# zju3dv/pats

Measured on AMD Instinct MI355X. Metric: image-pairs/sec (coarse+fine OT) on 640x480 MegaDepth; OT iters/sec per pair, higher is better.
Workload: dtype f32 (contractions: fp32 operands split into fp16 hi + lo, three exact-product MFMA passes, fp32 accumulate)

## Files before the change

include/pats_amd.h:

```cpp
#ifndef PATS_AMD_H
#define PATS_AMD_H

#include <stddef.h>
#include <stdint.h>

#ifdef __cplusplus
extern "C" {
#endif

typedef void* pats_stream_t;

enum {
    PATS_OK = 0,
    PATS_ERR_INVALID = 1,
    PATS_ERR_UNSUPPORTED = 2,
    PATS_ERR_LAUNCH = 3,
    PATS_ERR_NO_DEVICE = 4
};

enum { PATS_SINKHORN_AUTO = 0, PATS_SINKHORN_LOG = 1, PATS_SINKHORN_KERNEL = 2 };

const char* pats_version(void);
#define PATS_ABI_VERSION 8
int pats_abi_version(void);
const char* pats_last_error(void);
int pats_device_count(void);
int pats_set_sinkhorn_mode(int mode);
int pats_set_fine_fused(int on);

int pats_set_third_gather(int mode);

int pats_sinkhorn_fallbacks(int64_t* count, int reset);

int pats_cost_f32(const float* d0, const float* d1, int64_t batch, int D, int n, int m, float* out,
                  pats_stream_t stream);

size_t pats_sinkhorn_workspace_bytes(int64_t batch, int M, int N);
int pats_sinkhorn_f32(const float* Z, int64_t batch, int M, int N, const float* log_mu,
                      const float* log_nu, int iters, float* out, void* workspace,
                      size_t workspace_bytes, pats_stream_t stream);

size_t pats_ot_workspace_bytes(int64_t batch, int M, int N);
int pats_log_optimal_transport_f32(const float* scores, int64_t batch, int m, int n,
                                   const float* alpha, const float* ns, int iters, float* Z,
                                   void* workspace, size_t workspace_bytes, pats_stream_t stream);

size_t pats_ot2_workspace_bytes(int64_t batch, int m, int n);
int pats_log_optimal_transport2_flags_f32(const float* scores, int64_t batch, int m, int n,
                                          const float* one, const float* ns, int iters, float bias_k,
                                          float* Z, uint8_t* col_nomatch, void* workspace,
                                          size_t workspace_bytes, pats_stream_t stream);
int pats_log_optimal_transport2_f32(const float* scores, int64_t batch, int m, int n,
                                    const float* one, const float* ns, int iters, float bias_k,
                                    float* Z, void* workspace, size_t workspace_bytes,
                                    pats_stream_t stream);

int pats_cost_ot_f32(const float* d0, const float* d1, int64_t batch, int D, int n, int m,
                     int variant, const float* scalar, const float* ns, int iters, float bias_k,
                     float* Z, void* workspace, size_t workspace_bytes, pats_stream_t stream);
size_t pats_cost_ot_workspace_bytes(int64_t batch, int D, int n, int m, int variant);
int pats_cost_ot_flags_f32(const float* d0, const float* d1, int64_t batch, int D, int n, int m,
                           int variant, const float* scalar, const float* ns, int iters, float bias_k,
                           float* Z, uint8_t* col_nomatch, void* workspace, size_t workspace_bytes,
                           pats_stream_t stream);

int pats_set_cost_ot_mid_event(void* event);

int pats_cost_ot_flags_counted_f32(const float* d0, const float* d1, int64_t batch_cap, const int64_t* batch_dev,
                                   int D, int n, int m, int variant, const float* scalar, const float* ns, int iters,
                                   float bias_k, float* Z, uint8_t* col_nomatch, void* workspace,
                                   size_t workspace_bytes, pats_stream_t stream);

int pats_colmass_sqrt_f32(const float* Z, int64_t batch, int M, int N, float* out,
                          pats_stream_t stream);
int pats_colmass_flags_f32(const float* Z, int64_t batch, int M, int N, float* out, uint8_t* col_nomatch,
                           pats_stream_t stream);
int pats_dustbin_bias_inplace_f32(float* Z, int64_t batch, int M, int N, float k,
                                  pats_stream_t stream);
int pats_exp_f32(const float* Z, int64_t count, float* out, pats_stream_t stream);

int pats_argmax_f32(const float* Z, int64_t batch, int M, int N, int64_t* row_arg,
                    int64_t* col_arg, pats_stream_t stream);

int pats_iterative_expand_f32(const float* P, int input_is_log, int64_t batch, int M, int N,
                              const float* scalex, const float* scaley, int lim3, int h, int w,
                              float lower_bound, int iter_num, float* whole_cost, float* core_cost,
                              float* average_point, float* x_scale, float* y_scale, int64_t* bound,
                              uint8_t* row_nomatch, pats_stream_t stream);

int pats_iterative_expand_counted_f32(const float* P, int input_is_log, int64_t batch_cap, const int64_t* batch_dev,
                                      int M, int N, const float* scalex, const float* scaley, int lim3, int h, int w,
                                      float lower_bound, int iter_num, float* whole_cost, float* core_cost,
                                      float* average_point, float* x_scale, float* y_scale, int64_t* bound,
                                      uint8_t* row_nomatch, pats_stream_t stream);

int pats_split_patches(const int32_t* sum_cycle_host, int height, int width, int max_once_used,
                       int64_t* second_layer_set, int64_t* third_layer_set);
int pats_split_patches_device(const int32_t* sum_cycle, int64_t pairs, int height, int width,
                              int max_once_used, int64_t* second_layer_set, int64_t* third_layer_set,
                              int32_t* cycle_num, pats_stream_t stream);

int pats_compute_imgs_bounds_f32(const float* x_scale, const float* y_scale,
                                 const float* average_point, const uint8_t* if_nomatching, int Np,
                                 int height, int width, int img, int64_t* bound5, int64_t* K_out,
                                 float* x_scale_new, float* y_scale_new, float* average_new,
                                 pats_stream_t stream);

int pats_left_crops_f32(const float* left, int n_img, int H, int W, const int64_t* bound5, int64_t K,
                        int height, int width, float* out, pats_stream_t stream);

int pats_compute_imgs_bounds_batch_f32(const float* x_scale, const float* y_scale, const float* average_point,
                                       const uint8_t* if_nomatching, int n_img, int Np, int height, int width,
                                       int64_t* bound5, int64_t* K_img, int64_t* K_total, float* x_scale_new,
// ... 372 lines not shown
```

pats_amd/_lib.py:

```python
import ctypes
import os

_HERE = os.path.dirname(os.path.abspath(__file__))
LIB_PATH = os.path.join(_HERE, "libpats_amd.so")
if os.environ.get("PATS_AMD_DIAG_LIB", "") not in ("", "0"):
    _sfx = os.environ["PATS_AMD_DIAG_LIB"]
    LIB_PATH = os.path.join(_HERE, "libpats_amd_diag%s.so" % ("" if _sfx == "1" else _sfx))

c_void_p, c_int, c_i64, c_f, c_size = (ctypes.c_void_p, ctypes.c_int, ctypes.c_int64, ctypes.c_float,
                                       ctypes.c_size_t)

ABI_VERSION = 8



class PairTable(ctypes.Structure):
    _fields_ = [("pairs", ctypes.c_int64), ("shape_host", c_void_p), ("cell_base_host", c_void_p), ("shape", c_void_p),
                ("cell_base", c_void_p), ("img_base", c_void_p)]


_TAB = ctypes.POINTER(PairTable)


class CropFormat(ctypes.Structure):
    _fields_ = [("dtype", ctypes.c_int32), ("layout", ctypes.c_int32), ("normalize", ctypes.c_int32),
                ("mean", ctypes.c_float * 3), ("std", ctypes.c_float * 3)]


_FMT = ctypes.POINTER(CropFormat)

SIGNATURES = {
    "pats_version": (ctypes.c_char_p, []),
    "pats_abi_version": (c_int, []),
    "pats_last_error": (ctypes.c_char_p, []),
    "pats_device_count": (c_int, []),
    "pats_set_sinkhorn_mode": (c_int, [c_int]),
    "pats_set_fine_fused": (c_int, [c_int]),
    "pats_set_third_gather": (c_int, [c_int]),
    "pats_sinkhorn_fallbacks": (c_int, [ctypes.POINTER(ctypes.c_int64), c_int]),
    "pats_set_gnn_redo_mode": (c_int, [c_int]),
    "pats_gnn_overflows": (c_int, [ctypes.POINTER(ctypes.c_int64), c_int]),
    "pats_cost_f32": (c_int, [c_void_p, c_void_p, c_i64, c_int, c_int, c_int, c_void_p, c_void_p]),
    "pats_sinkhorn_workspace_bytes": (c_size, [c_i64, c_int, c_int]),
    "pats_sinkhorn_f32": (c_int, [c_void_p, c_i64, c_int, c_int, c_void_p, c_void_p, c_int, c_void_p,
                                  c_void_p, c_size, c_void_p]),
    "pats_ot_workspace_bytes": (c_size, [c_i64, c_int, c_int]),
    "pats_log_optimal_transport_f32": (c_int, [c_void_p, c_i64, c_int, c_int, c_void_p, c_void_p, c_int,
                                               c_void_p, c_void_p, c_size, c_void_p]),
    "pats_ot2_workspace_bytes": (c_size, [c_i64, c_int, c_int]),
    "pats_log_optimal_transport2_f32": (c_int, [c_void_p, c_i64, c_int, c_int, c_void_p, c_void_p, c_int,
                                                c_f, c_void_p, c_void_p, c_size, c_void_p]),
    "pats_cost_ot_f32": (c_int, [c_void_p, c_void_p, c_i64, c_int, c_int, c_int, c_int, c_void_p,
                                 c_void_p, c_int, c_f, c_void_p, c_void_p, c_size, c_void_p]),
    "pats_cost_ot_flags_f32": (c_int, [c_void_p, c_void_p, c_i64, c_int, c_int, c_int, c_int, c_void_p,
                                       c_void_p, c_int, c_f, c_void_p, c_void_p, c_void_p, c_size, c_void_p]),
    "pats_set_cost_ot_mid_event": (c_int, [c_void_p]),
    "pats_cost_ot_flags_counted_f32": (c_int, [c_void_p, c_void_p, c_i64, c_void_p, c_int, c_int, c_int, c_int, c_void_p,
                                               c_void_p, c_int, c_f, c_void_p, c_void_p, c_void_p, c_size, c_void_p]),
    "pats_iterative_expand_counted_f32": (c_int, [c_void_p, c_int, c_i64, c_void_p, c_int, c_int, c_void_p, c_void_p, c_int,
                                                  c_int, c_int, c_f, c_int, c_void_p, c_void_p, c_void_p,
                                                  c_void_p, c_void_p, c_void_p, c_void_p, c_void_p]),
    "pats_fine_descriptors_counted_f32": (c_int, [c_void_p, c_void_p, c_void_p, c_void_p, c_void_p, c_i64, c_void_p, c_int,
                                                  c_void_p, c_void_p]),
    "pats_log_optimal_transport2_flags_f32": (c_int, [c_void_p, c_i64, c_int, c_int, c_void_p, c_void_p, c_int,
                                                      c_f, c_void_p, c_void_p, c_void_p, c_size, c_void_p]),
    "pats_colmass_flags_f32": (c_int, [c_void_p, c_i64, c_int, c_int, c_void_p, c_void_p, c_void_p]),
    "pats_cost_ot_workspace_bytes": (c_size, [c_i64, c_int, c_int, c_int, c_int]),
    "pats_colmass_sqrt_f32": (c_int, [c_void_p, c_i64, c_int, c_int, c_void_p, c_void_p]),
    "pats_dustbin_bias_inplace_f32": (c_int, [c_void_p, c_i64, c_int, c_int, c_f, c_void_p]),
    "pats_exp_f32": (c_int, [c_void_p, c_i64, c_void_p, c_void_p]),
    "pats_argmax_f32": (c_int, [c_void_p, c_i64, c_int, c_int, c_void_p, c_void_p, c_void_p]),
    "pats_iterative_expand_f32": (c_int, [c_void_p, c_int, c_i64, c_int, c_int, c_void_p, c_void_p, c_int,
                                          c_int, c_int, c_f, c_int, c_void_p, c_void_p, c_void_p,
                                          c_void_p, c_void_p, c_void_p, c_void_p, c_void_p]),
    "pats_split_patches": (c_int, [c_void_p, c_int, c_int, c_int, c_void_p, c_void_p]),
    "pats_split_patches_device": (c_int, [c_void_p, c_i64, c_int, c_int, c_int, c_void_p, c_void_p, c_void_p, c_void_p]),
    "pats_compute_imgs_bounds_batch_f32": (c_int, [c_void_p, c_void_p, c_void_p, c_void_p, c_int, c_int, c_int, c_int,
                                                   c_void_p, c_void_p, c_void_p, c_void_p, c_void_p, c_void_p, c_void_p]),
    "pats_left_crops_counted_f32": (c_int, [c_void_p, c_int, c_int, c_int, c_void_p, c_i64, c_void_p, c_int, c_int,
                                            c_void_p, c_void_p]),
    "pats_tensor_resize_hwc_counted_f32": (c_int, [c_void_p, c_int, c_int, c_int, c_int, c_void_p, c_i64, c_void_p,
                                                   c_void_p, c_void_p, c_void_p]),
    "pats_compute_imgs_bounds_f32": (c_int, [c_void_p, c_void_p, c_void_p, c_void_p, c_int, c_int, c_int,
                                             c_int, c_void_p, c_void_p, c_void_p, c_void_p, c_void_p,
                                             c_void_p]),
    "pats_left_crops_f32": (c_int, [c_void_p, c_int, c_int, c_int, c_void_p, c_i64, c_int, c_int, c_void_p,
                                    c_void_p]),
    "pats_tensor_resize_f32": (c_int, [c_void_p, c_int, c_int, c_int, c_int, c_void_p, c_i64, c_void_p,
                                       c_void_p, c_void_p]),
    "pats_tensor_resize_hwc_f32": (c_int, [c_void_p, c_int, c_int, c_int, c_int, c_void_p, c_i64,
                                           c_void_p, c_void_p, c_void_p]),
    "pats_compute_result_f32": (c_int, [c_void_p, c_int, c_i64, c_void_p, c_void_p, c_void_p, c_void_p,
                                        c_int, c_void_p, c_void_p, c_void_p, c_void_p, c_void_p,
                                        c_void_p]),
    "pats_compute_result_ws_f32": (c_int, [c_void_p, c_int, c_i64, c_void_p, c_void_p, c_void_p, c_void_p,
                                           c_int, c_void_p, c_void_p, c_void_p, c_void_p, c_void_p,
                                           c_void_p, c_size, c_void_p]),
    "pats_fine_descriptors_f32": (c_int, [c_void_p, c_void_p, c_void_p, c_void_p, c_void_p, c_i64, c_void_p, c_void_p]),
    "pats_third_descriptors_f32": (c_int, [c_void_p, c_void_p, c_void_p, c_void_p, c_void_p, c_void_p, c_void_p,
                                           c_i64, c_i64, c_void_p, c_void_p, c_void_p, c_void_p, c_void_p]),
    "pats_third_level_f32": (c_int, [c_void_p, c_void_p, c_i64, c_int, c_void_p, c_void_p, c_void_p, c_void_p,
                                     c_void_p, c_int, c_int, c_void_p, c_void_p, c_void_p, c_void_p, c_void_p,
                                     c_void_p]),
    "pats_third_descriptors_counted_f32": (c_int, [c_void_p, c_void_p, c_void_p, c_void_p, c_void_p, c_void_p, c_void_p,
                                                   c_i64, c_void_p, c_i64, c_void_p, c_void_p, c_void_p, c_void_p, c_void_p]),
    "pats_fine_descriptors_nhwc_f32": (c_int, [c_void_p, c_void_p, c_void_p, c_void_p, c_void_p, c_i64, c_void_p, c_void_p]),
    "pats_third_descriptors_nhwc_f32": (c_int, [c_void_p, c_void_p, c_void_p, c_void_p, c_void_p, c_void_p, c_void_p,
                                                c_i64, c_void_p, c_i64, c_void_p, c_void_p, c_void_p, c_void_p, c_void_p]),
    "pats_fine_descriptors_typed": (c_int, [c_void_p, c_void_p, c_void_p, c_int, c_int, c_void_p, c_void_p, c_i64, c_void_p,
                                            c_void_p, c_void_p]),
    "pats_third_descriptors_typed": (c_int, [c_void_p, c_void_p, c_int, c_int, c_void_p, c_void_p, c_void_p, c_void_p, c_void_p,
                                             c_i64, c_void_p, c_i64, c_void_p, c_void_p, c_void_p, c_void_p, c_void_p]),
    "pats_fine_descriptors_typed_out": (c_int, [c_void_p, c_void_p, c_void_p, c_int, c_int, c_void_p, c_void_p, c_i64, c_void_p,
                                                c_void_p, c_int, c_void_p]),
    "pats_third_descriptors_typed_out": (c_int, [c_void_p, c_void_p, c_int, c_int, c_void_p, c_void_p, c_void_p, c_void_p,
                                                 c_void_p, c_i64, c_void_p, c_i64, c_void_p, c_void_p, c_int, c_void_p, c_void_p,
                                                 c_void_p]),
    "pats_third_level_counted_f32": (c_int, [c_void_p, c_void_p, c_i64, c_void_p, c_int, c_void_p, c_void_p, c_void_p,
                                             c_void_p, c_void_p, c_int, c_int, c_void_p, c_void_p, c_void_p, c_void_p,
                                             c_void_p]),
    "pats_cost_typed": (c_int, [c_void_p, c_void_p, c_int, c_i64, c_int, c_int, c_int, c_void_p, c_void_p]),
# ... 165 lines not shown
```

pats_amd/csrc/expand.hip:

```cpp
#include "common.hpp"
#include "third_device.hpp"

namespace pats {

struct ExpandArgs {
    const float* P;
    int input_is_log;
    int64_t rows_total;
    int M, N;
    const float* scalex;
    const float* scaley;
    int lim3, h, w;
    float lower_bound;
    int iter_num;
    float *whole_cost, *core_cost, *average_point, *x_scale, *y_scale;
    int64_t* bound;
    uint8_t* row_nomatch;
    const int64_t* live;
};

__device__ __forceinline__ float range_val(int d, int k) { return k <= d ? (float)k : 1e7f; }

__device__ __forceinline__ int clamp_seq(float f, int wh, int S) {
    return (f >= 0.f && f <= (float)(wh - 1)) ? (int)f : S;
}


template <bool SMALL>
__global__ void __launch_bounds__(256)
expand_kernel(ExpandArgs a) {
    extern __shared__ __attribute__((aligned(16))) float sm[];
    const int t = threadIdx.x & 15, slot = threadIdx.x >> 4;
    const int ROWS_PER_WG = blockDim.x >> 4;
    const int M = a.M, N = a.N, m = M - 1, n = N - 1;
    int64_t rows_total = a.rows_total;
    if (a.live) {
        const int64_t lv = *a.live * m;
        rows_total = lv < rows_total ? lv : rows_total;
        if ((int64_t)blockIdx.x * ROWS_PER_WG >= rows_total) return;
    }
    const int64_t gr_raw = (int64_t)blockIdx.x * ROWS_PER_WG + slot;
    const bool active = gr_raw < rows_total;
    const int64_t gr = active ? gr_raw : rows_total - 1;
    const int64_t b = gr / m;
    const int r = (int)(gr - b * m);
    const int ld = N + 3;
    float* prow = sm + (size_t)slot * ld;
    float* popp = sm + (size_t)ROWS_PER_WG * ld + (size_t)slot * ld;
    const float* Pb = a.P + b * (int64_t)M * N;
    const float* src = Pb + (int64_t)r * N;
    const float* oppsrc = Pb + (int64_t)(M - 1) * N;
    const float* sx = a.scalex + b * (int64_t)n;
    const float* sy = a.scaley + b * (int64_t)n;
    float fv = -INFINITY;
    int fi = 0x7fffffff;
    const int64_t g0 = (int64_t)blockIdx.x * ROWS_PER_WG;
    const int64_t glast = min(g0 + ROWS_PER_WG - 1, rows_total - 1);
    const int64_t b0 = g0 / m;
    const bool shared_opp = glast / m - b0 <= 1;
    if (shared_opp) {
        popp = sm + (size_t)ROWS_PER_WG * ld + (size_t)(b - b0) * ld;
        for (int e = threadIdx.x; e < 2 * N; e += blockDim.x) {
            const int which = e >= N, j = e - which * N;
            const int64_t bb = min(b0 + which, (int64_t)(rows_total - 1) / m);
            const float o = a.P[bb * (int64_t)M * N + (int64_t)(M - 1) * N + j];
            sm[(size_t)ROWS_PER_WG * ld + (size_t)which * ld + j] = a.input_is_log ? expf(o) : o;
        }
    }
    float bv = -INFINITY, bva = -INFINITY;
    int bi = 0x7fffffff, bia = 0x7fffffff;
    float rowsum = 0.f;
    for (int j = t; j < N; j += 16) {
        const float x0 = src[j];
        if (x0 > fv || fi == 0x7fffffff) { fv = x0; fi = j; }
        const float x = a.input_is_log ? expf(x0) : x0;
        prow[j] = x;
        rowsum += x;
        if (j < N - 1 && (x > bv || bi == 0x7fffffff)) { bv = x; bi = j; }
        if (x > bva || bia == 0x7fffffff) { bva = x; bia = j; }
        if (!shared_opp) {
            const float o = oppsrc[j];
            popp[j] = a.input_is_log ? expf(o) : o;
        }
    }
    if (a.row_nomatch) {
        row16_argmax(fv, fi);
        if (t == 0 && active) a.row_nomatch[gr] = fi == N - 1;
    }
    if (t == 0) { prow[N] = ZERO_F; popp[N] = ZERO_F; }
    wg_barrier();

    const int width = a.h > a.w ? a.h : a.w;
    const int height = (a.h * a.w) / width;
    const int wh = width * height, S = wh + 1;
    auto ES = [&](int idx) { return prow[idx]; };
    auto ESC = [&](int idx) { return idx < n ? sx[idx] * sy[idx] : ZERO_F; };
    auto EOPP = [&](int idx) { return popp[idx]; };

    row16_argmax(bv, bi);
    row16_argmax(bva, bia);
    const float the_scale = row16_sum(rowsum);
    const int max0 = bi;
    const bool if_nomatching = (bia == m);
    float last_nomatching = EOPP(max0);
    int up = max0 / a.lim3, down = up, left = max0 % a.lim3, right = left;
    int bd0 = 0, bd1 = 0, sb0 = 0, sb1 = 0;
    float last_sum = ES(max0);

    for (int it = 0; it < a.iter_num; ++it) {
        sb0 = bd0; sb1 = bd1;
        const float off[4] = {(float)(left + up * width - width),
                              (float)(left + down * width + width),
                              (float)(left + up * width - 1),
                              (float)(right + up * width + 1)};
        float es[4], nm[4], sc[4];
        float vcell[4];
        int scell[4];
#pragma unroll
        for (int d = 0; d < 4; ++d) {
            float e = 0.f, q = 0.f, c = 0.f;
            auto cell = [&](int k) {
                const float f = d < 2 ? range_val(sb1, k) + off[d] : range_val(sb0, k) * (float)width + off[d];
                const int s = clamp_seq(f, wh, S);
                const float v = ES(s);
                e += v;
                if (SMALL) { vcell[d] = v; scell[d] = s; }
                else {
                    q += (v > a.lower_bound) ? EOPP(s) : ZERO_F;
                    c += ESC(s);
                }
            };
            if (SMALL) { vcell[d] = 0.f; scell[d] = S; if (t < width) cell(t); }
            else for (int k = t; k < width; k += 16) cell(k);
            es[d] = row16_sum(e);
            if (!SMALL) { nm[d] = row16_sum(q); sc[d] = row16_sum(c); }
        }
        if (up == 0) es[0] = ZERO_F;
        if (down == height - 1) es[1] = ZERO_F;
        if (left == 0) es[2] = ZERO_F;
        if (right == width - 1) es[3] = ZERO_F;
        int arg = 0;
        float mx = es[0];
#pragma unroll
        for (int d = 1; d < 4; ++d)
            if (es[d] > mx) { mx = es[d]; arg = d; }
        float mnm;
        if (SMALL) {
            float v = vcell[0];
            int sidx = scell[0];
#pragma unroll
            for (int d = 1; d < 4; ++d)
                if (arg == d) { v = vcell[d]; sidx = scell[d]; }
            const float q = (t < width) ? ((v > a.lower_bound) ? EOPP(sidx) : ZERO_F) : 0.f;
            mnm = row16_sum(q);
        } else {
            mnm = nm[0];
#pragma unroll
            for (int d = 1; d < 4; ++d)
                if (arg == d) mnm = nm[d];
        }
        (void)sc;
        float add_sum = ZERO_F, add_nm = ZERO_F;
        if (mx > a.lower_bound) {
            up -= (arg == 0);
            down += (arg == 1);
            left -= (arg == 2);
            right += (arg == 3);
            add_sum = mx;
            add_nm = mnm;
        }
        bd0 = down - up;
        bd1 = right - left;
        last_sum = last_sum + add_sum;
        last_nomatching = last_nomatching + add_nm;
    }
    const bool if_core_exist = (bd0 > 1) && (bd1 > 1);

    float e4, s4;
    {
        const float eoff[4] = {(float)(left + up * width), (float)(left + down * width),
                               (float)(left + up * width), (float)(right + up * width)};
        float ed[4], sd[4];
#pragma unroll
        for (int d = 0; d < 4; ++d) {
            float e = 0.f, c = 0.f;
            auto cell = [&](int k) {
                const float f = d < 2 ? range_val(sb1, k) + eoff[d]
                                      : range_val(sb0, k) * (float)width + eoff[d];
                const int s = clamp_seq(f, wh, S);
                e += ES(s);
                c += ESC(s);
            };
            if (SMALL) { if (t < width) cell(t); }
            else for (int k = t; k < width; k += 16) cell(k);
            ed[d] = row16_sum(e);
            sd[d] = row16_sum(c);
        }
        e4 = (ed[0] + ed[1]) + (ed[2] + ed[3]);
        s4 = (sd[0] + sd[1]) + (sd[2] + sd[3]);
    }

    float wx = 0.f, wy = 0.f, sumx = 0.f, sumy = 0.f, ws = 0.f, so = 0.f;
    const int q16 = 16 / a.w, r16 = 16 - q16 * a.w;
    int pyi = t / a.w, pxi = t - pyi * a.w;
    const bool no_cell = up > (n - 1) / a.w || left > a.w - 1;
    for (int p = t; p < n; p += 16, pyi += q16, pxi += r16) {
        if (pxi >= a.w) { pxi -= a.w; ++pyi; }
        const bool crit = pyi >= up && pyi <= down && pxi >= left && pxi <= right;
        if (!__any(crit || no_cell)) continue;
        const float fx = sx[p], fy = sy[p];
        float ox = ZERO_F, oy = ZERO_F;
        if (crit) {
            const float root = sqrtf(prow[p] + 1e-7f);
            ox = root / fx;
            oy = root / fy;
        }
        wx += ox * (float)pxi;
        wy += oy * (float)pyi;
        sumx += ox;
        sumy += oy;
        const float o = ox * oy;
        ws += o * (fx * fy);
        so += o;
    }
    wx = row16_sum(wx); wy = row16_sum(wy); sumx = row16_sum(sumx); sumy = row16_sum(sumy);
    ws = row16_sum(ws); so = row16_sum(so);

    if (t == 0 && active) {
        const int corner[4] = {up * width + left, up * width + right, down * width + left,
                               down * width + right};
        float cps = 0.f, css = 0.f;
#pragma unroll
        for (int q = 0; q < 4; ++q) {
            int s = corner[q];
            if (!(s >= 0)) s = S;
            if (!(s <= wh - 1)) s = S;
            cps += ES(s);
            css += ESC(s);
        }
        const float core_scale_sum = the_scale - s4 + css;
        const float core_sum = last_sum - e4 + cps;
        a.core_cost[gr] = (if_core_exist && !if_nomatching)
                              ? fabsf((core_sum - core_scale_sum) / the_scale) : ZERO_F;
        a.whole_cost[gr] = if_nomatching ? ZERO_F
            : (fabsf(the_scale - last_sum) + last_nomatching / 4.0f) / the_scale;
        a.average_point[gr * 2 + 1] = wx / sumx + 0.5f;
        a.average_point[gr * 2 + 0] = wy / sumy + 0.5f;
        const float average_scale = sqrtf(ws / so);
        a.x_scale[gr] = 1.0f / (average_scale / 1.0f);
        a.y_scale[gr] = 1.0f / (average_scale * 1.0f);
        a.bound[gr * 4 + 0] = up;
        a.bound[gr * 4 + 1] = down;
        a.bound[gr * 4 + 2] = left;
        a.bound[gr * 4 + 3] = right;
    }
}

}

using namespace pats;

static int expand_impl(const float* P, int input_is_log, int64_t batch, int M, int N, const float* scalex, const float* scaley,
                       int lim3, int h, int w, float lower_bound, int iter_num, float* whole_cost, float* core_cost,
                       float* average_point, float* x_scale, float* y_scale, int64_t* bound, uint8_t* row_nomatch,
                       const int64_t* live, pats_stream_t stream);

extern "C" int pats_iterative_expand_f32(const float* P, int input_is_log, int64_t batch, int M,
                                         int N, const float* scalex, const float* scaley, int lim3,
                                         int h, int w, float lower_bound, int iter_num,
                                         float* whole_cost, float* core_cost, float* average_point,
                                         float* x_scale, float* y_scale, int64_t* bound,
                                         uint8_t* row_nomatch, pats_stream_t stream) {
    return expand_impl(P, input_is_log, batch, M, N, scalex, scaley, lim3, h, w, lower_bound, iter_num, whole_cost, core_cost,
                       average_point, x_scale, y_scale, bound, row_nomatch, nullptr, stream);
}

extern "C" int pats_iterative_expand_counted_f32(const float* P, int input_is_log, int64_t batch_cap, const int64_t* batch_dev,
                                                 int M, int N, const float* scalex, const float* scaley, int lim3, int h, int w,
                                                 float lower_bound, int iter_num, float* whole_cost, float* core_cost,
                                                 float* average_point, float* x_scale, float* y_scale, int64_t* bound,
                                                 uint8_t* row_nomatch, pats_stream_t stream) {
    PATS_REQUIRE(batch_dev, "iterative_expand_counted: null count");
    return expand_impl(P, input_is_log, batch_cap, M, N, scalex, scaley, lim3, h, w, lower_bound, iter_num, whole_cost, core_cost,
                       average_point, x_scale, y_scale, bound, row_nomatch, batch_dev, stream);
}

static int expand_impl(const float* P, int input_is_log, int64_t batch, int M, int N, const float* scalex, const float* scaley,
                       int lim3, int h, int w, float lower_bound, int iter_num, float* whole_cost, float* core_cost,
                       float* average_point, float* x_scale, float* y_scale, int64_t* bound, uint8_t* row_nomatch,
                       const int64_t* live, pats_stream_t stream) {
    PATS_REQUIRE(batch >= 0 && M > 1 && N > 1 && h > 0 && w > 0 && lim3 > 0 && iter_num >= 1,
                 "iterative_expand: bad argument");
    PATS_REQUIRE(h * w == N - 1, "iterative_expand: grid %dx%d does not match %d target columns", h,
                 w, N - 1);
    if (batch == 0) return PATS_OK;
    PATS_REQUIRE(P && scalex && scaley && whole_cost && core_cost && average_point && x_scale &&
                     y_scale && bound, "iterative_expand: null pointer");
    ExpandArgs a{P, input_is_log, batch * (int64_t)(M - 1), M, N, scalex, scaley, lim3, h, w,
                 lower_bound, iter_num, whole_cost, core_cost, average_point, x_scale, y_scale, bound, row_nomatch, live};
    int rows_per_wg = 16;
    size_t lds = 2 * (size_t)rows_per_wg * (size_t)(N + 3) * sizeof(float);
    if (lds > 48 * 1024) {
        rows_per_wg = 4;
        lds = 2 * (size_t)rows_per_wg * (size_t)(N + 3) * sizeof(float);
    }
    PATS_REQUIRE(lds <= 64 * 1024, "iterative_expand: N=%d too large", N);
    const int64_t blocks = ceil_div(a.rows_total, rows_per_wg);
    if (h <= 16 && w <= 16)
        hipLaunchKernelGGL(expand_kernel<true>, dim3((unsigned)blocks), dim3(16 * rows_per_wg), lds, as_stream(stream), a);
    else
        hipLaunchKernelGGL(expand_kernel<false>, dim3((unsigned)blocks), dim3(16 * rows_per_wg), lds, as_stream(stream), a);
    return check_launch("expand_kernel");
}
```

pats_amd/ops.py:

```python
import ctypes

import numpy as np
import torch

from . import _lib

_L = _lib.lib
_check = _lib.check
_L()


_raw_stream = getattr(torch._C, "_cuda_getCurrentRawStream", None)


def _stream():
    if _raw_stream is not None:
        return ctypes.c_void_p(_raw_stream(torch.cuda.current_device()))
    return ctypes.c_void_p(torch.cuda.current_stream().cuda_stream)


def _dev(t, name, dtype=torch.float32):
    if not isinstance(t, torch.Tensor):
        raise TypeError("%s must be a torch.Tensor" % name)
    if not t.is_cuda:
# ... 27 lines not shown
            raise RuntimeError("pats_amd: %s must be float32, float16 or bfloat16, got %s" % (name, t.dtype))
    dtypes = {t.dtype for t in tensors}
    if dtypes == {torch.float32}:
        return [_map(t, n) for t, n in zip(tensors, names)], _MAP_DTYPES[torch.float32]
    if len(dtypes) != 1:
        return [_map(t.float(), n) for t, n in zip(tensors, names)], _MAP_DTYPES[torch.float32]
    dt = tensors[0].dtype
    maps = [_map(t, n, dt) for t, n in zip(tensors, names)]
    if len({cl for _, cl in maps}) != 1:
        maps = [(t.contiguous(), False) for t, _ in maps]
    align = 16 if maps[0][1] else 4
    if any(t.data_ptr() % align for t, _ in maps):
        return [_map(t.float(), n) for t, n in zip(tensors, names)], _MAP_DTYPES[torch.float32]
    return maps, _MAP_DTYPES[dt]


def _descs_any(tensors, names):
    for t, name in zip(tensors, names):
        if not isinstance(t, torch.Tensor):
            raise TypeError("%s must be a torch.Tensor" % name)
        if t.dtype not in _MAP_DTYPES:
            raise RuntimeError("pats_amd: %s must be float32, float16 or bfloat16, got %s" % (name, t.dtype))
    dtypes = {t.dtype for t in tensors}
    if len(dtypes) == 1 and torch.float32 not in dtypes:
        dt = tensors[0].dtype
        descs = [_dev(t, n, dt) for t, n in zip(tensors, names)]
        if not any(t.data_ptr() % t.element_size() for t in descs):
            return descs, _MAP_DTYPES[dt]
    return [_dev(t.float(), n) for t, n in zip(tensors, names)], _MAP_DTYPES[torch.float32]


def _ptr(t):
    return ctypes.c_void_p(t.data_ptr()) if t is not None else ctypes.c_void_p(0)


_WS = {}
_WS_MAX = 64 << 20
_WS_ON = [False]


class workspace_cache:

    def __enter__(self):
        self.prev = _WS_ON[0]
        _WS_ON[0] = True

    def __exit__(self, *exc):
        _WS_ON[0] = self.prev


def _workspace(nbytes, device):
    n = max(int(nbytes), 1)
    if not _WS_ON[0] or n > _WS_MAX or _raw_stream is None or torch.cuda.is_current_stream_capturing():
        return torch.empty(n, dtype=torch.uint8, device=device)
    key = (device.index, _raw_stream(torch.cuda.current_device()))
    t = _WS.get(key)
    if t is None or t.numel() < n:
        t = _WS[key] = torch.empty(min(_WS_MAX, max(2 * n, 1 << 20)), dtype=torch.uint8, device=device)
    return t


def _scalar_dev(x, device):
    if isinstance(x, torch.Tensor):
        return x.detach().reshape(1).to(device=device, dtype=torch.float32)
    return torch.full((1,), float(x), dtype=torch.float32, device=device)


def set_sinkhorn_mode(mode):
    names = {"auto": 0, "log": 1, "kernel": 2}
    prev = _L().pats_set_sinkhorn_mode(names[mode])
    return {v: k for k, v in names.items()}[prev]


def set_fine_fused(on):
    return bool(_L().pats_set_fine_fused(1 if on else 0))


def set_third_gather(mode):
    modes = {"tile": 0, "point": 1}
    if mode not in modes:
        raise ValueError("set_third_gather: mode must be 'tile' or 'point'")
    prev = _L().pats_set_third_gather(modes[mode])
    return {v: k for k, v in modes.items()}.get(prev, "tile")


def sinkhorn_fallbacks(reset=True):
    import ctypes
    n = ctypes.c_int64(0)
    rc = _L().pats_sinkhorn_fallbacks(ctypes.byref(n), 1 if reset else 0)
    if rc != 0:
        raise RuntimeError(_L().pats_last_error().decode())
    return int(n.value)


def set_gnn_redo(mode):
    names = {"inline": 0, "deferred": 1}
    prev = _L().pats_set_gnn_redo_mode(names[mode])
    return {v: k for k, v in names.items()}[prev]


def gnn_overflows(reset=True):
    n = ctypes.c_int64(0)
    _check(_L().pats_gnn_overflows(ctypes.byref(n), 1 if reset else 0), "gnn_overflows")
    return bool(n.value)


def cost(mdesc0, mdesc1, out=None):
    (d0, d1), code = _descs_any([mdesc0, mdesc1], ["mdesc0", "mdesc1"])
    b, D, n = d0.shape
    if d1.shape[0] != b or d1.shape[1] != D:
        raise RuntimeError("cost: descriptor shapes %s / %s do not match" % (tuple(d0.shape), tuple(d1.shape)))
    m = d1.shape[2]
    if out is None:
        out = torch.empty((b, n, m), dtype=torch.float32, device=d0.device)
    elif tuple(out.shape) != (b, n, m) or out.dtype != torch.float32 or not out.is_contiguous() or out.device != d0.device:
        raise RuntimeError("cost: out must be a contiguous float32 [%d, %d, %d] tensor on %s" % (b, n, m, d0.device))
    if code:
        _check(_L().pats_cost_typed(_ptr(d0), _ptr(d1), code, b, D, n, m, _ptr(out), _stream()), "cost")
    else:
        _check(_L().pats_cost_f32(_ptr(d0), _ptr(d1), b, D, n, m, _ptr(out), _stream()), "cost")
    return out


def log_sinkhorn_iterations(Z, log_mu, log_nu, iters: int):
    Z, log_mu, log_nu = _dev(Z, "Z"), _dev(log_mu, "log_mu"), _dev(log_nu, "log_nu")
    b, M, N = Z.shape
    if tuple(log_mu.shape) != (b, M) or tuple(log_nu.shape) != (b, N):
        raise RuntimeError("log_sinkhorn_iterations: marginal shapes do not match Z")
    out = torch.empty_like(Z)
    nb = _L().pats_sinkhorn_workspace_bytes(b, M, N)
    ws = _workspace(nb, Z.device)
    _check(_L().pats_sinkhorn_f32(_ptr(Z), b, M, N, _ptr(log_mu), _ptr(log_nu), int(iters), _ptr(out),
                                  _ptr(ws), nb, _stream()), "log_sinkhorn_iterations")
    return out


def log_optimal_transport(scores, alpha, ns, iters: int):
    scores = _dev(scores, "scores")
    b, m, n = scores.shape
    ns = _dev(ns, "ns")
    if ns.numel() != b * n:
        raise RuntimeError("log_optimal_transport: ns must have %d entries per batch" % n)
    ns = ns.reshape(b, n)
    a = _scalar_dev(alpha, scores.device)
    Z = torch.empty((b, m + 1, n + 1), dtype=torch.float32, device=scores.device)
    nb = _L().pats_ot_workspace_bytes(b, m + 1, n + 1)
    ws = _workspace(nb, scores.device)
    _check(_L().pats_log_optimal_transport_f32(_ptr(scores), b, m, n, _ptr(a), _ptr(ns), int(iters),
                                               _ptr(Z), _ptr(ws), nb, _stream()), "log_optimal_transport")
    return Z


def log_optimal_transport2(scores, one, ns, iters: int, bias_k: float = 0.0):
    scores = _dev(scores, "scores")
    b, m, n = scores.shape
    ns = _dev(ns, "ns")
    if ns.numel() != b * (n - 1):
        raise RuntimeError("log_optimal_transport2: ns must have %d entries per batch" % (n - 1))
    ns = ns.reshape(b, n - 1)
    o = _scalar_dev(one, scores.device)
    Z = torch.empty((b, m, n), dtype=torch.float32, device=scores.device)
    nb = _L().pats_ot2_workspace_bytes(b, m, n)
    ws = _workspace(nb, scores.device)
    _check(_L().pats_log_optimal_transport2_f32(_ptr(scores), b, m, n, _ptr(o), _ptr(ns), int(iters),
                                                float(bias_k), _ptr(Z), _ptr(ws), nb, _stream()),
           "log_optimal_transport2")
# ... 1814 lines not shown
```

Baseline: 1939.

## Process expand rows with 4-lane quads and exit early once the region stops growing

Moves the iterative-expand body into a shared header and adds a 4-lane-per-row variant for small grids, selected by default. Each 64-thread slice of a wave now covers 16 rows, reducing with quad DPP and sharing one dust row. The growth loop also stops once the whole wave's regions stop changing, padding the skipped iterations with the zero increment to keep the sums matching. The aim is to cut idle lanes and wasted iterations, at the cost of more work per lane and more LDS per workgroup.

```diff
diff --git a/include/pats_amd.h b/include/pats_amd.h
--- a/include/pats_amd.h
+++ b/include/pats_amd.h
@@ -29,6 +29,8 @@
 int pats_set_fine_fused(int on);
 
 int pats_set_third_gather(int mode);
+
+int pats_set_expand_lanes(int lanes);
 
 int pats_sinkhorn_fallbacks(int64_t* count, int reset);
 
diff --git a/pats_amd/_lib.py b/pats_amd/_lib.py
--- a/pats_amd/_lib.py
+++ b/pats_amd/_lib.py
@@ -37,6 +37,7 @@
     "pats_set_sinkhorn_mode": (c_int, [c_int]),
     "pats_set_fine_fused": (c_int, [c_int]),
     "pats_set_third_gather": (c_int, [c_int]),
+    "pats_set_expand_lanes": (c_int, [c_int]),
     "pats_sinkhorn_fallbacks": (c_int, [ctypes.POINTER(ctypes.c_int64), c_int]),
     "pats_set_gnn_redo_mode": (c_int, [c_int]),
     "pats_gnn_overflows": (c_int, [ctypes.POINTER(ctypes.c_int64), c_int]),
diff --git a/pats_amd/csrc/expand.hip b/pats_amd/csrc/expand.hip
--- a/pats_amd/csrc/expand.hip
+++ b/pats_amd/csrc/expand.hip
@@ -1,38 +1,65 @@
+#include <type_traits>
 #include "common.hpp"
 #include "third_device.hpp"
+#include "expand_body.hpp"
+
+#ifndef PATS_EXPAND_OPT
+#define PATS_EXPAND_OPT EXPAND_OPT_FIXED_EXIT
+#endif
 
 namespace pats {
 
+static_assert(EXPAND_ZERO == ZERO_F, "expand_body.hpp carries its own copy of the reference's zero");
+
 struct ExpandArgs {
     const float* P;
-    int input_is_log;
     int64_t rows_total;
-    int M, N;
+    ExpandShape s;
     const float* scalex;
     const float* scaley;
-    int lim3, h, w;
-    float lower_bound;
-    int iter_num;
     float *whole_cost, *core_cost, *average_point, *x_scale, *y_scale;
     int64_t* bound;
     uint8_t* row_nomatch;
     const int64_t* live;
 };
 
-__device__ __forceinline__ float range_val(int d, int k) { return k <= d ? (float)k : 1e7f; }
+struct ExpandRow16 {
+    static constexpr int G = 16;
+    int t;
+    __device__ __forceinline__ float sum(float v) const { return row16_sum(v); }
+    __device__ __forceinline__ void argmax(float& v, int& i) const { row16_argmax(v, i); }
+    __device__ __forceinline__ bool any_rows(bool p) const { return __any(p); }
+    __device__ __forceinline__ bool all_wave(bool p) const { return __all(p); }
+};
 
-__device__ __forceinline__ int clamp_seq(float f, int wh, int S) {
-    return (f >= 0.f && f <= (float)(wh - 1)) ? (int)f : S;
-}
+struct ExpandQuad4 {
+    static constexpr int G = 4;
+    int t;
+    __device__ __forceinline__ float sum(float v) const {
+        v += dpp_f<DPP_QUAD_XOR1>(v);
+        v += dpp_f<DPP_QUAD_XOR2>(v);
+        return v;
+    }
+    __device__ __forceinline__ void argmax(float& v, int& i) const {
+        argmax_step<DPP_QUAD_XOR1>(v, i);
+        argmax_step<DPP_QUAD_XOR2>(v, i);
+    }
+    __device__ __forceinline__ bool any_rows(bool p) const {
+        const unsigned long long bal = __ballot(p);
+        return ((bal >> (threadIdx.x & 48)) & 0xffffull) != 0;
+    }
+    __device__ __forceinline__ bool all_wave(bool p) const { return __all(p); }
+};
 
-
-template <bool SMALL>
+template <bool SMALL, int G = 16>
 __global__ void __launch_bounds__(256)
 expand_kernel(ExpandArgs a) {
     extern __shared__ __attribute__((aligned(16))) float sm[];
-    const int t = threadIdx.x & 15, slot = threadIdx.x >> 4;
-    const int ROWS_PER_WG = blockDim.x >> 4;
-    const int M = a.M, N = a.N, m = M - 1, n = N - 1;
+    using Grp = typename std::conditional<G == 16, ExpandRow16, ExpandQuad4>::type;
+    const Grp g{(int)(threadIdx.x & (G - 1))};
+    const int t = g.t, slot = threadIdx.x / G;
+    const int ROWS_PER_WG = blockDim.x / G;
+    const int M = a.s.M, N = a.s.N, m = M - 1, n = N - 1;
     int64_t rows_total = a.rows_total;
     if (a.live) {
         const int64_t lv = *a.live * m;
@@ -46,213 +73,50 @@
     const int r = (int)(gr - b * m);
     const int ld = N + 3;
     float* prow = sm + (size_t)slot * ld;
-    float* popp = sm + (size_t)ROWS_PER_WG * ld + (size_t)slot * ld;
+    float* dust = sm + (size_t)ROWS_PER_WG * ld;
+    float* popp = dust + (size_t)slot * ld;
     const float* Pb = a.P + b * (int64_t)M * N;
     const float* src = Pb + (int64_t)r * N;
     const float* oppsrc = Pb + (int64_t)(M - 1) * N;
     const float* sx = a.scalex + b * (int64_t)n;
     const float* sy = a.scaley + b * (int64_t)n;
-    float fv = -INFINITY;
-    int fi = 0x7fffffff;
     const int64_t g0 = (int64_t)blockIdx.x * ROWS_PER_WG;
     const int64_t glast = min(g0 + ROWS_PER_WG - 1, rows_total - 1);
     const int64_t b0 = g0 / m;
-    const bool shared_opp = glast / m - b0 <= 1;
+    const bool shared_opp = G == 4 || glast / m - b0 <= 1;
     if (shared_opp) {
-        popp = sm + (size_t)ROWS_PER_WG * ld + (size_t)(b - b0) * ld;
+        popp = dust + (size_t)(b - b0) * ld;
         for (int e = threadIdx.x; e < 2 * N; e += blockDim.x) {
             const int which = e >= N, j = e - which * N;
             const int64_t bb = min(b0 + which, (int64_t)(rows_total - 1) / m);
             const float o = a.P[bb * (int64_t)M * N + (int64_t)(M - 1) * N + j];
-            sm[(size_t)ROWS_PER_WG * ld + (size_t)which * ld + j] = a.input_is_log ? expf(o) : o;
+            dust[(size_t)which * ld + j] = a.s.input_is_log ? expf(o) : o;
+        }
+    } else {
+        for (int j = t; j < N; j += G) {
+            const float o = oppsrc[j];
+            popp[j] = a.s.input_is_log ? expf(o) : o;
         }
     }
-    float bv = -INFINITY, bva = -INFINITY;
-    int bi = 0x7fffffff, bia = 0x7fffffff;
-    float rowsum = 0.f;
-    for (int j = t; j < N; j += 16) {
-        const float x0 = src[j];
-        if (x0 > fv || fi == 0x7fffffff) { fv = x0; fi = j; }
-        const float x = a.input_is_log ? expf(x0) : x0;
-        prow[j] = x;
-        rowsum += x;
-        if (j < N - 1 && (x > bv || bi == 0x7fffffff)) { bv = x; bi = j; }
-        if (x > bva || bia == 0x7fffffff) { bva = x; bia = j; }
-        if (!shared_opp) {
-            const float o = oppsrc[j];
-            popp[j] = a.input_is_log ? expf(o) : o;
-        }
-    }
-    if (a.row_nomatch) {
-        row16_argmax(fv, fi);
-        if (t == 0 && active) a.row_nomatch[gr] = fi == N - 1;
-    }
+    const ExpandLane st = expand_stage(g, a.s, src, prow);
     if (t == 0) { prow[N] = ZERO_F; popp[N] = ZERO_F; }
     wg_barrier();
 
-    const int width = a.h > a.w ? a.h : a.w;
-    const int height = (a.h * a.w) / width;
-    const int wh = width * height, S = wh + 1;
-    auto ES = [&](int idx) { return prow[idx]; };
-    auto ESC = [&](int idx) { return idx < n ? sx[idx] * sy[idx] : ZERO_F; };
-    auto EOPP = [&](int idx) { return popp[idx]; };
-
-    row16_argmax(bv, bi);
-    row16_argmax(bva, bia);
-    const float the_scale = row16_sum(rowsum);
-    const int max0 = bi;
-    const bool if_nomatching = (bia == m);
-    float last_nomatching = EOPP(max0);
-    int up = max0 / a.lim3, down = up, left = max0 % a.lim3, right = left;
-    int bd0 = 0, bd1 = 0, sb0 = 0, sb1 = 0;
-    float last_sum = ES(max0);
-
-    for (int it = 0; it < a.iter_num; ++it) {
-        sb0 = bd0; sb1 = bd1;
-        const float off[4] = {(float)(left + up * width - width),
-                              (float)(left + down * width + width),
-                              (float)(left + up * width - 1),
-                              (float)(right + up * width + 1)};
-        float es[4], nm[4], sc[4];
-        float vcell[4];
-        int scell[4];
-#pragma unroll
-        for (int d = 0; d < 4; ++d) {
-            float e = 0.f, q = 0.f, c = 0.f;
-            auto cell = [&](int k) {
-                const float f = d < 2 ? range_val(sb1, k) + off[d] : range_val(sb0, k) * (float)width + off[d];
-                const int s = clamp_seq(f, wh, S);
-                const float v = ES(s);
-                e += v;
-                if (SMALL) { vcell[d] = v; scell[d] = s; }
-                else {
-                    q += (v > a.lower_bound) ? EOPP(s) : ZERO_F;
-                    c += ESC(s);
-                }
-            };
-            if (SMALL) { vcell[d] = 0.f; scell[d] = S; if (t < width) cell(t); }
-            else for (int k = t; k < width; k += 16) cell(k);
-            es[d] = row16_sum(e);
-            if (!SMALL) { nm[d] = row16_sum(q); sc[d] = row16_sum(c); }
-        }
-        if (up == 0) es[0] = ZERO_F;
-        if (down == height - 1) es[1] = ZERO_F;
-        if (left == 0) es[2] = ZERO_F;
-        if (right == width - 1) es[3] = ZERO_F;
-        int arg = 0;
-        float mx = es[0];
-#pragma unroll
-        for (int d = 1; d < 4; ++d)
-            if (es[d] > mx) { mx = es[d]; arg = d; }
-        float mnm;
-        if (SMALL) {
-            float v = vcell[0];
-            int sidx = scell[0];
-#pragma unroll
-            for (int d = 1; d < 4; ++d)
-                if (arg == d) { v = vcell[d]; sidx = scell[d]; }
-            const float q = (t < width) ? ((v > a.lower_bound) ? EOPP(sidx) : ZERO_F) : 0.f;
-            mnm = row16_sum(q);
-        } else {
-            mnm = nm[0];
-#pragma unroll
-            for (int d = 1; d < 4; ++d)
-                if (arg == d) mnm = nm[d];
-        }
-        (void)sc;
-        float add_sum = ZERO_F, add_nm = ZERO_F;
-        if (mx > a.lower_bound) {
-            up -= (arg == 0);
-            down += (arg == 1);
-            left -= (arg == 2);
-            right += (arg == 3);
-            add_sum = mx;
-            add_nm = mnm;
-        }
-        bd0 = down - up;
-        bd1 = right - left;
-        last_sum = last_sum + add_sum;
-        last_nomatching = last_nomatching + add_nm;
-    }
-    const bool if_core_exist = (bd0 > 1) && (bd1 > 1);
-
-    float e4, s4;
-    {
-        const float eoff[4] = {(float)(left + up * width), (float)(left + down * width),
-                               (float)(left + up * width), (float)(right + up * width)};
-        float ed[4], sd[4];
-#pragma unroll
-        for (int d = 0; d < 4; ++d) {
-            float e = 0.f, c = 0.f;
-            auto cell = [&](int k) {
-                const float f = d < 2 ? range_val(sb1, k) + eoff[d]
-                                      : range_val(sb0, k) * (float)width + eoff[d];
-                const int s = clamp_seq(f, wh, S);
-                e += ES(s);
-                c += ESC(s);
-            };
-            if (SMALL) { if (t < width) cell(t); }
-            else for (int k = t; k < width; k += 16) cell(k);
-            ed[d] = row16_sum(e);
-            sd[d] = row16_sum(c);
-        }
-        e4 = (ed[0] + ed[1]) + (ed[2] + ed[3]);
-        s4 = (sd[0] + sd[1]) + (sd[2] + sd[3]);
-    }
-
-    float wx = 0.f, wy = 0.f, sumx = 0.f, sumy = 0.f, ws = 0.f, so = 0.f;
-    const int q16 = 16 / a.w, r16 = 16 - q16 * a.w;
-    int pyi = t / a.w, pxi = t - pyi * a.w;
-    const bool no_cell = up > (n - 1) / a.w || left > a.w - 1;
-    for (int p = t; p < n; p += 16, pyi += q16, pxi += r16) {
-        if (pxi >= a.w) { pxi -= a.w; ++pyi; }
-        const bool crit = pyi >= up && pyi <= down && pxi >= left && pxi <= right;
-        if (!__any(crit || no_cell)) continue;
-        const float fx = sx[p], fy = sy[p];
-        float ox = ZERO_F, oy = ZERO_F;
-        if (crit) {
-            const float root = sqrtf(prow[p] + 1e-7f);
-            ox = root / fx;
-            oy = root / fy;
-        }
-        wx += ox * (float)pxi;
-        wy += oy * (float)pyi;
-        sumx += ox;
-        sumy += oy;
-        const float o = ox * oy;
-        ws += o * (fx * fy);
-        so += o;
-    }
-    wx = row16_sum(wx); wy = row16_sum(wy); sumx = row16_sum(sumx); sumy = row16_sum(sumy);
-    ws = row16_sum(ws); so = row16_sum(so);
+    ExpandResult o;
+    expand_grow<Grp, SMALL, PATS_EXPAND_OPT>(g, a.s, prow, popp, sx, sy, st, o);
 
     if (t == 0 && active) {
-        const int corner[4] = {up * width + left, up * width + right, down * width + left,
-                               down * width + right};
-        float cps = 0.f, css = 0.f;
-#pragma unroll
-        for (int q = 0; q < 4; ++q) {
-            int s = corner[q];
-            if (!(s >= 0)) s = S;
-            if (!(s <= wh - 1)) s = S;
-            cps += ES(s);
-            css += ESC(s);
-        }
-        const float core_scale_sum = the_scale - s4 + css;
-        const float core_sum = last_sum - e4 + cps;
-        a.core_cost[gr] = (if_core_exist && !if_nomatching)
-                              ? fabsf((core_sum - core_scale_sum) / the_scale) : ZERO_F;
-        a.whole_cost[gr] = if_nomatching ? ZERO_F
-            : (fabsf(the_scale - last_sum) + last_nomatching / 4.0f) / the_scale;
-        a.average_point[gr * 2 + 1] = wx / sumx + 0.5f;
-        a.average_point[gr * 2 + 0] = wy / sumy + 0.5f;
-        const float average_scale = sqrtf(ws / so);
-        a.x_scale[gr] = 1.0f / (average_scale / 1.0f);
-        a.y_scale[gr] = 1.0f / (average_scale * 1.0f);
-        a.bound[gr * 4 + 0] = up;
-        a.bound[gr * 4 + 1] = down;
-        a.bound[gr * 4 + 2] = left;
-        a.bound[gr * 4 + 3] = right;
+        if (a.row_nomatch) a.row_nomatch[gr] = o.nomatch;
+        a.core_cost[gr] = o.core_cost;
+        a.whole_cost[gr] = o.whole_cost;
+        a.average_point[gr * 2 + 1] = o.avg_x;
+        a.average_point[gr * 2 + 0] = o.avg_y;
+        a.x_scale[gr] = o.x_scale;
+        a.y_scale[gr] = o.y_scale;
+        a.bound[gr * 4 + 0] = o.up;
+        a.bound[gr * 4 + 1] = o.down;
+        a.bound[gr * 4 + 2] = o.left;
+        a.bound[gr * 4 + 3] = o.right;
     }
 }
 
@@ -285,6 +149,16 @@
                        average_point, x_scale, y_scale, bound, row_nomatch, batch_dev, stream);
 }
 
+#ifndef PATS_EXPAND_LANES
+#define PATS_EXPAND_LANES 4
+#endif
+static int g_expand_lanes = PATS_EXPAND_LANES;
+extern "C" int pats_set_expand_lanes(int lanes) {
+    const int prev = g_expand_lanes;
+    if (lanes == 4 || lanes == 16) g_expand_lanes = lanes;
+    return prev;
+}
+
 static int expand_impl(const float* P, int input_is_log, int64_t batch, int M, int N, const float* scalex, const float* scaley,
                        int lim3, int h, int w, float lower_bound, int iter_num, float* whole_cost, float* core_cost,
                        float* average_point, float* x_scale, float* y_scale, int64_t* bound, uint8_t* row_nomatch,
@@ -296,8 +170,19 @@
     if (batch == 0) return PATS_OK;
     PATS_REQUIRE(P && scalex && scaley && whole_cost && core_cost && average_point && x_scale &&
                      y_scale && bound, "iterative_expand: null pointer");
-    ExpandArgs a{P, input_is_log, batch * (int64_t)(M - 1), M, N, scalex, scaley, lim3, h, w,
-                 lower_bound, iter_num, whole_cost, core_cost, average_point, x_scale, y_scale, bound, row_nomatch, live};
+    ExpandArgs a{P, batch * (int64_t)(M - 1), ExpandShape{M, N, lim3, h, w, iter_num, lower_bound, input_is_log, row_nomatch != nullptr},
+                 scalex, scaley, whole_cost, core_cost, average_point, x_scale, y_scale, bound, row_nomatch, live};
+    const bool small = h <= 16 && w <= 16;
+    if (small && g_expand_lanes == 4) {
+        int rows4 = 64;
+        if ((size_t)(rows4 + 2) * (size_t)(N + 3) * sizeof(float) > 48 * 1024) rows4 = 32;
+        const size_t lds4 = (size_t)(rows4 + 2) * (size_t)(N + 3) * sizeof(float);
+        if (M - 1 >= rows4 && lds4 <= 48 * 1024) {
+            hipLaunchKernelGGL((expand_kernel<true, 4>), dim3((unsigned)ceil_div(a.rows_total, rows4)), dim3(4 * rows4), lds4,
+                               as_stream(stream), a);
+            return check_launch("expand_kernel");
+        }
+    }
     int rows_per_wg = 16;
     size_t lds = 2 * (size_t)rows_per_wg * (size_t)(N + 3) * sizeof(float);
     if (lds > 48 * 1024) {
@@ -306,7 +191,7 @@
     }
     PATS_REQUIRE(lds <= 64 * 1024, "iterative_expand: N=%d too large", N);
     const int64_t blocks = ceil_div(a.rows_total, rows_per_wg);
-    if (h <= 16 && w <= 16)
+    if (small)
         hipLaunchKernelGGL(expand_kernel<true>, dim3((unsigned)blocks), dim3(16 * rows_per_wg), lds, as_stream(stream), a);
     else
         hipLaunchKernelGGL(expand_kernel<false>, dim3((unsigned)blocks), dim3(16 * rows_per_wg), lds, as_stream(stream), a);
diff --git a/pats_amd/csrc/expand_body.hpp b/pats_amd/csrc/expand_body.hpp
--- /dev/null
+++ b/pats_amd/csrc/expand_body.hpp
@@ -0,0 +1,324 @@
+#pragma once
+#include <math.h>
+#include <stdint.h>
+
+#if defined(__HIPCC__)
+#define PATS_EXPAND_HD __host__ __device__ __forceinline__
+#else
+#define PATS_EXPAND_HD inline
+#endif
+
+namespace pats {
+
+constexpr float EXPAND_ZERO = 1e-14f;
+constexpr int EXPAND_NOIDX = 0x7fffffff;
+
+constexpr int EXPAND_OPT_FIXED_EXIT = 1;
+constexpr int EXPAND_OPT_STRIP_REUSE = 2;
+
+struct ExpandShape {
+    int M, N, lim3, h, w, iter_num;
+    float lower_bound;
+    int input_is_log;
+    int want_flag;
+};
+
+struct ExpandLane {
+    float fv; int fi;
+    float bv; int bi;
+    float bva; int bia;
+    float rowsum;
+};
+
+struct ExpandResult {
+    float whole_cost, core_cost, avg_y, avg_x, x_scale, y_scale;
+    int up, down, left, right;
+    int nomatch;
+};
+
+PATS_EXPAND_HD void expand_take(float& v, int& i, float ov, int oi) {
+    if (ov > v || (ov == v && oi < i)) { v = ov; i = oi; }
+}
+
+template <int V>
+PATS_EXPAND_HD float expand_fold(const float (&p)[V]) {
+    if constexpr (V == 1) return p[0];
+    else return (p[0] + p[1]) + (p[2] + p[3]);
+}
+
+template <int V>
+PATS_EXPAND_HD void expand_fold_best(float (&v)[V], int (&i)[V]) {
+    if constexpr (V == 4) {
+        expand_take(v[0], i[0], v[1], i[1]);
+        expand_take(v[2], i[2], v[3], i[3]);
+        expand_take(v[0], i[0], v[2], i[2]);
+    }
+}
+
+PATS_EXPAND_HD int expand_cell(int k, int span, int stride, int off, int wh, int S) {
+    const int s = k * stride + off;
+    return (k <= span && (unsigned)s < (unsigned)wh) ? s : S;
+}
+
+template <class Grp>
+PATS_EXPAND_HD ExpandLane expand_stage(const Grp& g, const ExpandShape& a, const float* src, float* prow) {
+    constexpr int V = 16 / Grp::G;
+    const int N = a.N;
+    float fv[V], bv[V], bva[V], rs[V];
+    int fi[V], bi[V], bia[V];
+#pragma unroll
+    for (int i = 0; i < V; ++i) {
+        fv[i] = bv[i] = bva[i] = -INFINITY;
+        fi[i] = bi[i] = bia[i] = EXPAND_NOIDX;
+        rs[i] = 0.f;
+    }
+    for (int j0 = g.t * V; j0 < N; j0 += 16) {
+#pragma unroll
+        for (int i = 0; i < V; ++i) {
+            const int j = j0 + i;
+            if (j < N) {
+                const float x0 = src[j];
+                if (x0 > fv[i] || fi[i] == EXPAND_NOIDX) { fv[i] = x0; fi[i] = j; }
+                const float x = a.input_is_log ? expf(x0) : x0;
+                prow[j] = x;
+                rs[i] += x;
+                if (j < N - 1 && (x > bv[i] || bi[i] == EXPAND_NOIDX)) { bv[i] = x; bi[i] = j; }
+                if (x > bva[i] || bia[i] == EXPAND_NOIDX) { bva[i] = x; bia[i] = j; }
+            }
+        }
+    }
+    expand_fold_best<V>(fv, fi);
+    expand_fold_best<V>(bv, bi);
+    expand_fold_best<V>(bva, bia);
+    return ExpandLane{fv[0], fi[0], bv[0], bi[0], bva[0], bia[0], expand_fold<V>(rs)};
+}
+
+template <class Grp, bool SMALL, int OPT>
+PATS_EXPAND_HD void expand_grow(const Grp& g, const ExpandShape& a, const float* prow, const float* popp, const float* sx,
+                                const float* sy, ExpandLane st, ExpandResult& out) {
+    constexpr int V = 16 / Grp::G;
+    constexpr float Z = EXPAND_ZERO;
+    const int N = a.N, m = a.M - 1, n = N - 1;
+    const int vl0 = g.t * V;
+    const int width = a.h > a.w ? a.h : a.w;
+    const int height = (a.h * a.w) / width;
+    const int wh = width * height, S = wh + 1;
+    auto ESC = [&](int idx) { return idx < n ? sx[idx] * sy[idx] : Z; };
+
+    if (a.want_flag) g.argmax(st.fv, st.fi);
+    g.argmax(st.bv, st.bi);
+    g.argmax(st.bva, st.bia);
+    const float the_scale = g.sum(st.rowsum);
+    const int max0 = st.bi;
+    const bool if_nomatching = (st.bia == m);
+    float last_nomatching = popp[max0];
+    int up = max0 / a.lim3, down = up, left = max0 % a.lim3, right = left;
+    int bd0 = 0, bd1 = 0, sb0 = 0, sb1 = 0;
+    float last_sum = prow[max0];
+
+    float raw[4], nm[4];
+    float vcell[4][V];
+    int scell[4][V];
+    int poff[4] = {0, 0, 0, 0}, pspan[4] = {-1, -1, -1, -1};
+    int it = 0;
+    for (; it < a.iter_num; ++it) {
+        sb0 = bd0; sb1 = bd1;
+        const int off[4] = {left + up * width - width,
+                            left + down * width + width,
+                            left + up * width - 1,
+                            right + up * width + 1};
+#pragma unroll
+        for (int d = 0; d < 4; ++d) {
+            const int span = d < 2 ? sb1 : sb0, stride = d < 2 ? 1 : width;
+            if ((OPT & EXPAND_OPT_STRIP_REUSE) && off[d] == poff[d] && span == pspan[d]) continue;
+            poff[d] = off[d];
+            pspan[d] = span;
+            float e[V], q[V];
+#pragma unroll
+            for (int i = 0; i < V; ++i) {
+                const int vl = vl0 + i;
+                e[i] = 0.f;
+                q[i] = 0.f;
+                if (SMALL) {
+                    vcell[d][i] = 0.f;
+                    scell[d][i] = S;
+                    if (vl < width) {
+                        const int s = expand_cell(vl, span, stride, off[d], wh, S);
+                        const float v = prow[s];
+                        e[i] += v;
+                        vcell[d][i] = v;
+                        scell[d][i] = s;
+                    }
+                } else {
+                    for (int k = vl; k < width; k += 16) {
+                        const int s = expand_cell(k, span, stride, off[d], wh, S);
+                        const float v = prow[s];
+                        e[i] += v;
+                        q[i] += (v > a.lower_bound) ? popp[s] : Z;
+                    }
+                }
+            }
+            raw[d] = g.sum(expand_fold<V>(e));
+            if (!SMALL) nm[d] = g.sum(expand_fold<V>(q));
+        }
+        float es[4] = {raw[0], raw[1], raw[2], raw[3]};
+        if (up == 0) es[0] = Z;
+        if (down == height - 1) es[1] = Z;
+        if (left == 0) es[2] = Z;
+        if (right == width - 1) es[3] = Z;
+        int arg = 0;
+        float mx = es[0];
+#pragma unroll
+        for (int d = 1; d < 4; ++d)
+            if (es[d] > mx) { mx = es[d]; arg = d; }
+        float mnm;
+        if (SMALL) {
+            float q[V];
+#pragma unroll
+            for (int i = 0; i < V; ++i) {
+                float v = vcell[0][i];
+                int sidx = scell[0][i];
+#pragma unroll
+                for (int d = 1; d < 4; ++d)
+                    if (arg == d) { v = vcell[d][i]; sidx = scell[d][i]; }
+                q[i] = (vl0 + i < width) ? ((v > a.lower_bound) ? popp[sidx] : Z) : 0.f;
+            }
+            mnm = g.sum(expand_fold<V>(q));
+        } else {
+            mnm = nm[0];
+#pragma unroll
+            for (int d = 1; d < 4; ++d)
+                if (arg == d) mnm = nm[d];
+        }
+        float add_sum = Z, add_nm = Z;
+        const bool grow = mx > a.lower_bound;
+        if (grow) {
+            up -= (arg == 0);
+            down += (arg == 1);
+            left -= (arg == 2);
+            right += (arg == 3);
+            add_sum = mx;
+            add_nm = mnm;
+        }
+        bd0 = down - up;
+        bd1 = right - left;
+        last_sum = last_sum + add_sum;
+        last_nomatching = last_nomatching + add_nm;
+        if (OPT & EXPAND_OPT_FIXED_EXIT) {
+            if (g.all_wave(!grow && sb0 == bd0 && sb1 == bd1)) { ++it; break; }
+        }
+    }
+    for (; it < a.iter_num; ++it) {
+        last_sum = last_sum + Z;
+        last_nomatching = last_nomatching + Z;
+    }
+    const bool if_core_exist = (bd0 > 1) && (bd1 > 1);
+
+    float e4, s4;
+    {
+        const int eoff[4] = {left + up * width, left + down * width, left + up * width, right + up * width};
+        float ed[4], sd[4];
+#pragma unroll
+        for (int d = 0; d < 4; ++d) {
+            const int span = d < 2 ? sb1 : sb0, stride = d < 2 ? 1 : width;
+            float e[V], c[V];
+#pragma unroll
+            for (int i = 0; i < V; ++i) {
+                const int vl = vl0 + i;
+                e[i] = 0.f;
+                c[i] = 0.f;
+                if (SMALL) {
+                    if (vl < width) {
+                        const int s = expand_cell(vl, span, stride, eoff[d], wh, S);
+                        e[i] += prow[s];
+                        c[i] += ESC(s);
+                    }
+                } else {
+                    for (int k = vl; k < width; k += 16) {
+                        const int s = expand_cell(k, span, stride, eoff[d], wh, S);
+                        e[i] += prow[s];
+                        c[i] += ESC(s);
+                    }
+                }
+            }
+            ed[d] = g.sum(expand_fold<V>(e));
+            sd[d] = g.sum(expand_fold<V>(c));
+        }
+        e4 = (ed[0] + ed[1]) + (ed[2] + ed[3]);
+        s4 = (sd[0] + sd[1]) + (sd[2] + sd[3]);
+    }
+
+    float wx[V], wy[V], sumx[V], sumy[V], ws[V], so[V];
+    int pyi[V], pxi[V];
+    const int q16 = 16 / a.w, r16 = 16 - q16 * a.w;
+#pragma unroll
+    for (int i = 0; i < V; ++i) {
+        wx[i] = wy[i] = sumx[i] = sumy[i] = ws[i] = so[i] = 0.f;
+        pyi[i] = (vl0 + i) / a.w;
+        pxi[i] = (vl0 + i) - pyi[i] * a.w;
+    }
+    const bool no_cell = up > (n - 1) / a.w || left > a.w - 1;
+    for (int p0 = 0; p0 < n; p0 += 16) {
+        bool crit[V], need = false;
+#pragma unroll
+        for (int i = 0; i < V; ++i) {
+            if (pxi[i] >= a.w) { pxi[i] -= a.w; ++pyi[i]; }
+            const bool live = p0 + vl0 + i < n;
+            crit[i] = live && pyi[i] >= up && pyi[i] <= down && pxi[i] >= left && pxi[i] <= right;
+            need = need || (live && (crit[i] || no_cell));
+        }
+        if (g.any_rows(need)) {
+#pragma unroll
+            for (int i = 0; i < V; ++i) {
+                const int p = p0 + vl0 + i;
+                if (p < n) {
+                    const float fx = sx[p], fy = sy[p];
+                    float ox = Z, oy = Z;
+                    if (crit[i]) {
+                        const float root = sqrtf(prow[p] + 1e-7f);
+                        ox = root / fx;
+                        oy = root / fy;
+                    }
+                    wx[i] += ox * (float)pxi[i];
+                    wy[i] += oy * (float)pyi[i];
+                    sumx[i] += ox;
+                    sumy[i] += oy;
+                    const float o = ox * oy;
+                    ws[i] += o * (fx * fy);
+                    so[i] += o;
+                }
+            }
+        }
+#pragma unroll
+        for (int i = 0; i < V; ++i) { pyi[i] += q16; pxi[i] += r16; }
+    }
+    const float WX = g.sum(expand_fold<V>(wx)), WY = g.sum(expand_fold<V>(wy));
+    const float SX = g.sum(expand_fold<V>(sumx)), SY = g.sum(expand_fold<V>(sumy));
+    const float WS = g.sum(expand_fold<V>(ws)), SO = g.sum(expand_fold<V>(so));
+
+    if (g.t == 0) {
+        const int corner[4] = {up * width + left, up * width + right, down * width + left, down * width + right};
+        float cps = 0.f, css = 0.f;
+#pragma unroll
+        for (int q = 0; q < 4; ++q) {
+            int s = corner[q];
+            if (!(s >= 0)) s = S;
+            if (!(s <= wh - 1)) s = S;
+            cps += prow[s];
+            css += ESC(s);
+        }
+        const float core_scale_sum = the_scale - s4 + css;
+        const float core_sum = last_sum - e4 + cps;
+        out.core_cost = (if_core_exist && !if_nomatching) ? fabsf((core_sum - core_scale_sum) / the_scale) : Z;
+        out.whole_cost = if_nomatching ? Z : (fabsf(the_scale - last_sum) + last_nomatching / 4.0f) / the_scale;
+        out.avg_x = WX / SX + 0.5f;
+        out.avg_y = WY / SY + 0.5f;
+        const float average_scale = sqrtf(WS / SO);
+        out.x_scale = 1.0f / (average_scale / 1.0f);
+        out.y_scale = 1.0f / (average_scale * 1.0f);
+        out.up = up; out.down = down; out.left = left; out.right = right;
+        out.nomatch = st.fi == N - 1;
+    }
+}
+
+}
diff --git a/pats_amd/ops.py b/pats_amd/ops.py
--- a/pats_amd/ops.py
+++ b/pats_amd/ops.py
@@ -133,6 +133,12 @@
         raise ValueError("set_third_gather: mode must be 'tile' or 'point'")
     prev = _L().pats_set_third_gather(modes[mode])
     return {v: k for k, v in modes.items()}.get(prev, "tile")
+
+
+def set_expand_lanes(lanes):
+    if lanes not in (4, 16):
+        raise ValueError("set_expand_lanes: lanes must be 4 or 16")
+    return int(_L().pats_set_expand_lanes(int(lanes)))
 
 
 def sinkhorn_fallbacks(reset=True):
```

New measurement: 1936. No clear change (-0.1%).
